# NikolausDemmel/rootba

Measured on NVIDIA H100. Metric: ms/LM-iter (linearize+QR+PCG) on BAL at 1/2/4/8 H100 vs CPU ref, lower is better.
Workload: dtype f32

## Files before the change

rootba_b200/csrc/assembled.cuh:

```cuda
#pragma once

#include "kernels.cuh"

namespace rba {

template <class S>
__global__ void __launch_bounds__(256) k_rcs_terms(const S* __restrict__ panel, const AsmTerm* __restrict__ terms, long long nt,
                                                   int damping, S* __restrict__ stage, const int* __restrict__ done) {
  using V2 = typename ST<S>::V2;
  if (*done) return;
  const int lane = threadIdx.x & 31;
  const int g = lane / 9, p = lane - 9 * g;
  if (lane >= 27) return;
  const long long warps = (long long)gridDim.x * (blockDim.x >> 5);
  for (long long w = 3 * (blockIdx.x * (long long)(blockDim.x >> 5) + (threadIdx.x >> 5)) + g; w < nt; w += 3 * warps) {
    const AsmTerm at = terms[w];
    const int n = at.meta & 0x7fff, lg = (at.meta >> 15) & 7, KP = at.meta >> 18, G = 1 << lg;
    const int ia = at.ij & 0xffff, ib = at.ij >> 16;
    const int ca = 9 * ia + p, pa = ca >> 1;
    const int off_a = 2 * ((pa >> lg) * 32 + (pa & (G - 1))) + (ca & 1);
    const int cb0 = 9 * ib, pb0 = cb0 >> 1;
    const bool odd = cb0 & 1;
    int off_b[5];
#pragma unroll
    for (int k = 0; k < 5; ++k) off_b[k] = ((pb0 + k) >> lg) * 32 + ((pb0 + k) & (G - 1));
    const size_t rstride = (size_t)KP * 64;
    const S* __restrict__ lmp = panel + at.base;
    const int r0 = damping ? 2 * n - 3 : 0, r1 = damping ? 2 * n : 2 * n - 3;
    S acc[9];
#pragma unroll
    for (int q = 0; q < 9; ++q) acc[q] = 0;
#pragma unroll 3
    for (int r = r0; r < r1; ++r) {
      const S* row = lmp + (size_t)r * rstride;
      const V2* row2 = reinterpret_cast<const V2*>(row);
      const S va = __ldg(row + off_a);
      V2 b[5];
#pragma unroll
      for (int k = 0; k < 5; ++k) b[k] = __ldg(row2 + off_b[k]);
      const S el[10] = {b[0].x, b[0].y, b[1].x, b[1].y, b[2].x, b[2].y, b[3].x, b[3].y, b[4].x, b[4].y};
#pragma unroll
      for (int q = 0; q < 9; ++q) acc[q] = fma(va, odd ? el[q + 1] : el[q], acc[q]);
    }
    S* o = stage + 81 * (size_t)w + 9 * p;
#pragma unroll
    for (int q = 0; q < 9; ++q) o[q] = acc[q];
  }
}

template <class S>
__global__ void k_rcs_combine(const int* __restrict__ blk_ptr, const int* __restrict__ wpos, int nblk, const S* __restrict__ stage,
                              S* __restrict__ out, const int* __restrict__ done) {
  if (*done) return;
  const long long i = blockIdx.x * (long long)blockDim.x + threadIdx.x;
  if (i >= 81LL * nblk) return;
  const int bi = (int)(i / 81), e = (int)(i - 81LL * bi);
  const S* st = stage + e;
  S s = 0;
  for (int t = blk_ptr[bi]; t < blk_ptr[bi + 1]; ++t) s += st[81 * (size_t)wpos[t]];
  out[i] = s;
}

constexpr int DMP_WARPS = 4;
constexpr int DMP_BATCH = 16;
template <class S>
__global__ void __launch_bounds__(DMP_WARPS * 32) k_rcs_damping(const int* __restrict__ blk_ptr, const int2* __restrict__ terms, int nblk,
                                                                 const S* __restrict__ dmp, const S* __restrict__ base,
                                                                 const int2* __restrict__ pos, S* __restrict__ out,
                                                                 const int* __restrict__ done) {
  constexpr int B = DMP_BATCH, NV = 28 * sizeof(S) / 16;
  constexpr int ROUNDS = (2 * B * NV + 31) / 32;
  __shared__ __align__(16) S rec[DMP_WARPS][B][2][28];
  if (*done) return;
  const int w = threadIdx.x >> 5, lane = threadIdx.x & 31;
  const int bi = blockIdx.x * DMP_WARPS + w;
  if (bi >= nblk) return;
  const bool own = lane < 27;
  const int p = lane / 3, q = 3 * (lane - 3 * p);
  S s[3] = {0, 0, 0};
  if (own) {
#pragma unroll
    for (int u = 0; u < 3; ++u) s[u] = base[81 * (size_t)bi + 3 * lane + u];
  }
  int4* rv = reinterpret_cast<int4*>(&rec[w][0][0][0]);
  const int t1 = blk_ptr[bi + 1];
  for (int t0 = blk_ptr[bi]; t0 < t1; t0 += B) {
    const int nb = min(B, t1 - t0);
    int4 v[ROUNDS];
#pragma unroll
    for (int c = 0; c < ROUNDS; ++c) {
      const int i = lane + 32 * c, r = i / NV, k = i - r * NV;
      v[c] = make_int4(0, 0, 0, 0);
      if (i < 2 * nb * NV) {
        const int2 tt = __ldg(terms + t0 + (r >> 1));
        v[c] = __ldg(reinterpret_cast<const int4*>(dmp + 28 * (size_t)(r & 1 ? tt.y : tt.x)) + k);
      }
    }
#pragma unroll
    for (int c = 0; c < ROUNDS; ++c)
      if (lane + 32 * c < 2 * nb * NV) rv[lane + 32 * c] = v[c];
    __syncwarp();
    if (own) {
      for (int j = 0; j < nb; ++j) {
        const S* a = rec[w][j][0];
        const S* b = rec[w][j][1];
#pragma unroll
        for (int u = 0; u < 3; ++u) {
          S t = fma(a[p], b[q + u], S(0));
          t = fma(a[9 + p], b[9 + q + u], t);
          t = fma(a[18 + p], b[18 + q + u], t);
          s[u] += t;
        }
      }
    }
    __syncwarp();
  }
  if (own) {
    S* o = out + 81 * (size_t)pos[bi].x + 3 * lane;
#pragma unroll
    for (int u = 0; u < 3; ++u) o[u] = s[u];
  }
}

template <class S>
__global__ void k_rcs_mirror(const int2* __restrict__ pos, int nblk, S* val, const int* __restrict__ done) {
  if (*done) return;
  const long long i = blockIdx.x * (long long)blockDim.x + threadIdx.x;
  if (i >= 81LL * nblk) return;
  const int bi = (int)(i / 81), e = (int)(i - 81LL * bi);
// ... 140 lines not shown
```

rootba_b200/csrc/layout.hpp:

```cpp
#pragma once

#include <algorithm>
#include <cmath>
#include <cstdint>
#include <limits>
#include <numeric>
#include <string>
#include <utility>
#include <vector>

namespace rba {

struct TileInfo {
  long long panel_off;
  int slot_base;
  int lm_base;
  short n;
  short G;
  short KP;
  short nvalid;
};

struct MatvecItem {
  int tile;
// ... 237 lines not shown
    if (!L.csr_y_is_obs) build_csr(nc, L.nyslots, ycam, L.csr_y);
    L.pb_cam_item_ptr.assign(nc + 1, 0);
    for (int c = 0; c < nc; ++c) {
      L.pb_cam_item_ptr[c] = (int)L.pb_items.size();
      for (int b = L.csr_obs.cam_ptr[c]; b < L.csr_obs.cam_ptr[c + 1]; b += PB_SEG_LEN)
        L.pb_items.push_back({c, b, std::min(b + PB_SEG_LEN, L.csr_obs.cam_ptr[c + 1])});
    }
    L.pb_cam_item_ptr[nc] = (int)L.pb_items.size();
  }
  for (const TileInfo& T : L.tiles) {
    const int W = 32 / T.G;
    const int CS = (2 * T.G * T.KP) | 1;
    L.k4_scratch_per_warp = std::max(L.k4_scratch_per_warp, T.KP > kp_max ? 2 * 64 * (int)T.KP : W * CS);
  }
  return "";
}

struct IntPair {
  int x, y;
};

struct PairList {
  std::vector<int> slot0, nn;
  std::vector<IntPair> blk_cam;
  std::vector<int> blk_ptr;
  std::vector<IntPair> terms;
  std::vector<int> wpos;
};

inline std::string build_pair_list(const Layout& L, PairList& P) {
  const int nl = L.nl_local, nc = L.nc;
  P = PairList();
  P.slot0.resize(nl); P.nn.resize(nl);
  long long nt = 0;
  for (int lm = 0; lm < nl; ++lm) {
    const int sidx = L.sorted_of_lm[lm];
    const TileInfo& T = L.tiles[L.tile_of_sorted[sidx]];
    P.slot0[lm] = T.slot_base + (sidx - T.lm_base) * T.n;
    P.nn[lm] = T.n;
    nt += (long long)T.n * (T.n + 1) / 2;
  }
  if (nt > std::numeric_limits<int>::max()) return "more than 2^31 camera-pair terms";
  std::vector<IntPair> raw;
  raw.reserve((size_t)nt);
  for (int lm = 0; lm < nl; ++lm)
    for (int a = 0; a < P.nn[lm]; ++a)
      for (int b = 0; b <= a; ++b) raw.push_back({P.slot0[lm] + a, P.slot0[lm] + b});
  std::vector<int> idx(raw.size()), tmp(raw.size());
  std::iota(idx.begin(), idx.end(), 0);
  std::vector<long long> cnt((size_t)nc + 1);
  auto pass = [&](const std::vector<int>& src, std::vector<int>& dst, bool by_a) {
    std::fill(cnt.begin(), cnt.end(), 0LL);
    for (int w : src) ++cnt[L.slot_cam[by_a ? raw[w].x : raw[w].y] + 1];
    for (int c = 0; c < nc; ++c) cnt[c + 1] += cnt[c];
    for (int w : src) dst[cnt[L.slot_cam[by_a ? raw[w].x : raw[w].y]]++] = w;
  };
  pass(idx, tmp, false);
  pass(tmp, idx, true);
  tmp.clear(); tmp.shrink_to_fit();
  P.terms.resize(raw.size());
  for (size_t t = 0; t < idx.size(); ++t) P.terms[t] = raw[idx[t]];
  P.wpos.swap(idx);
  for (size_t t = 0; t < P.terms.size(); ++t) {
    const IntPair cc{L.slot_cam[P.terms[t].x], L.slot_cam[P.terms[t].y]};
    if (t == 0 || cc.x != P.blk_cam.back().x || cc.y != P.blk_cam.back().y) {
      P.blk_cam.push_back(cc);
      P.blk_ptr.push_back((int)t);
    }
  }
  P.blk_ptr.push_back((int)P.terms.size());
  return "";
}

struct AsmTerm {
  long long base;
  int ij, meta;
};
inline AsmTerm pack_asm_term(long long base, int ia, int ib, int n, int G, int KP) {
  int lg = 0;
  while ((1 << lg) < G) ++lg;
  return {base, ia | ib << 16, n | lg << 15 | KP << 18};
}

constexpr long long ASM_STAGE_BYTES = (long long)2 << 30;

inline int asm_switch_iteration(long long nt, long long panel_scalars, long long s_bytes, int scalar_size) {
  const double staged = 4.0 * (double)nt * 81 * scalar_size, saved = (double)panel_scalars * scalar_size - (double)s_bytes;
  return 1 + (int)std::ceil(2.0 * staged / std::max(saved, 1.0));
}

constexpr int SPMV_CLASSES = 4;
constexpr int SPMV_STAGE_BYTES = 32 * 81 * 4;
constexpr int spmv_chunk_blocks(int scalar_size) { return SPMV_STAGE_BYTES / (81 * scalar_size); }
struct SpmvChunk {
  int row, kb, ke;
  int flags;
};
constexpr int SPMV_FIRST = 1, SPMV_LAST = 2;
struct SpmvDeal {
  int ctas = 0;
  std::vector<int> chunk_ptr;
  std::vector<SpmvChunk> chunks;
};
inline void deal_spmv(const std::vector<int>& row_ptr, int ctas, int chunk_blocks, SpmvDeal& D) {
  D = SpmvDeal();
  const int nrows = (int)row_ptr.size() - 1;
  D.ctas = std::max(1, std::min(ctas, nrows));
  std::vector<long long> cost((size_t)std::max(nrows, 0));
  for (int r = 0; r < nrows; ++r) cost[r] = row_ptr[r + 1] - row_ptr[r];
  const std::vector<int> order = deal_lpt(cost, D.ctas);
  D.chunk_ptr.assign((size_t)D.ctas + 1, 0);
  for (int b = 0; b < D.ctas; ++b) {
    D.chunk_ptr[b] = (int)D.chunks.size();
    for (size_t k = b; k < order.size(); k += D.ctas) {
      const int r = order[k];
      if (r < 0) break;
      const int k0 = row_ptr[r], k1 = row_ptr[r + 1];
      int kb = k0;
      do {
        const int ke = std::min(k1, kb + chunk_blocks);
        D.chunks.push_back({r, kb, ke, (kb == k0 ? SPMV_FIRST : 0) | (ke == k1 ? SPMV_LAST : 0)});
        kb = ke;
      } while (kb < k1);
    }
  }
  D.chunk_ptr[D.ctas] = (int)D.chunks.size();
}

struct AsmPlan {
  long long nt = 0, nblk = 0, nnzb = 0, s_bytes = 0, device_bytes = 0;
  bool fits = false;
  int switch_iteration = 0;
  std::vector<int> row_ptr;
  std::vector<int> col;
  std::vector<IntPair> pos;
  std::vector<AsmTerm> terms;
  SpmvDeal spmv;
};

inline void plan_assembled(const Layout& L, const PairList& P, int scalar_size, AsmPlan& A, int spmv_ctas = 0) {
  A = AsmPlan();
  const int nc = L.nc;
  A.nblk = (long long)P.blk_cam.size();
  A.nt = (long long)P.terms.size();
  long long ndiag = 0;
  for (const IntPair& c : P.blk_cam) ndiag += c.x == c.y;
  A.nnzb = 2 * A.nblk - ndiag;
  A.s_bytes = A.nnzb * 81 * scalar_size;
  A.switch_iteration = asm_switch_iteration(A.nt, L.panel_scalars, A.s_bytes, scalar_size);
  A.fits = 4 * A.s_bytes <= L.panel_scalars * scalar_size && 81 * A.nt * scalar_size <= ASM_STAGE_BYTES;
  if (!A.fits) return;
  A.device_bytes = A.s_bytes + 16 + (A.nblk + A.nt) * 81 * scalar_size + A.nt * (long long)(sizeof(AsmTerm) + sizeof(int) + sizeof(IntPair)) +
                   (A.nblk + 1 + A.nnzb) * (long long)sizeof(int) + A.nblk * (long long)sizeof(IntPair);
  A.row_ptr.assign((size_t)nc + 1, 0);
  A.col.resize((size_t)A.nnzb);
  for (const IntPair& c : P.blk_cam) { ++A.row_ptr[c.x + 1]; if (c.x != c.y) ++A.row_ptr[c.y + 1]; }
  for (int c = 0; c < nc; ++c) A.row_ptr[c + 1] += A.row_ptr[c];
  std::vector<int> fill(A.row_ptr.begin(), A.row_ptr.end() - 1);
  A.pos.resize((size_t)A.nblk);
  for (long long b = 0; b < A.nblk; ++b) {
    const IntPair c = P.blk_cam[b];
    const int lo = fill[c.x]++;
    A.col[lo] = c.y;
    int up = -1;
    if (c.x != c.y) { up = fill[c.y]++; A.col[up] = c.x; }
    A.pos[b] = {lo, up};
  }
  A.terms.reserve((size_t)A.nt);
  for (int lm = 0; lm < L.nl_local; ++lm) {
    const int sidx = L.sorted_of_lm[lm];
    const TileInfo& T = L.tiles[L.tile_of_sorted[sidx]];
    const int g = sidx - T.lm_base;
    for (int a = 0; a < T.n; ++a)
      for (int b = 0; b <= a; ++b) A.terms.push_back(pack_asm_term(T.panel_off + 2LL * g * T.G, a, b, T.n, T.G, T.KP));
  }
  if (spmv_ctas > 0) {
    deal_spmv(A.row_ptr, spmv_ctas, spmv_chunk_blocks(scalar_size), A.spmv);
    A.device_bytes += (long long)A.spmv.chunks.size() * (long long)sizeof(SpmvChunk) + (A.spmv.ctas + 1) * (long long)sizeof(int);
  }
}

}
```

rootba_b200/csrc/solver.cu:

```cuda
#include <cuda_runtime.h>
#include <dlfcn.h>

#include <cstdio>
#include <cstdlib>
#include <cstring>
#include <chrono>
#include <array>
#include <limits>
#include <memory>
#include <string>
#include <utility>
#include <vector>

#include "../../include/rootba_b200.h"
#include "../host/bal_io_fast.hpp"
#include "kernels.cuh"
#include "covariance.cuh"
#include "assembled.cuh"
#include "rigs.cuh"
#include "nccl_dyn.hpp"

namespace rba {

thread_local std::string g_err;
// ... 47 lines not shown
  virtual int set_intrinsics_groups(const int32_t* group) = 0;
  virtual int set_camera_rigs(const int32_t* rig, const void* cam_from_rig) = 0;
  virtual int set_observation_info(const void* sqrt_info) = 0;
  virtual int set_observation_loss(const uint8_t* kind, const void* scale) = 0;
  virtual int set_prior_loss(int32_t prior_kind, int32_t num, const uint8_t* kind, const void* scale) = 0;
  virtual int get_prior_residuals(int32_t prior_kind, void* residual, void* robust_weight) = 0;
  virtual int get_observation_residuals(void* residual, void* robust_weight, uint8_t* flags) = 0;
  virtual int compute_error(rba_residual_info* out) = 0;
  virtual int linearize() = 0;
  virtual int solve(double lambda, void* inc_out, rba_cg_summary* cg) = 0;
  virtual int apply(const void* inc, void* l_diff_out, bool update_cameras) = 0;
  virtual int lm_step(bool linearize_first, double lambda, rba_lm_step_result* out) = 0;
  virtual int lm_run(const rba_lm_opts* o, int max_steps, rba_lm_iteration* log, int* steps_done, int* terminated, rba_stage_timings* totals) = 0;
  virtual int get_timings(rba_stage_timings* out) const = 0;
  virtual int get_stats(rba_workload_stats* out) const = 0;
  virtual int get_scaling(void* scaling, void* diag2) = 0;
  virtual int get_rhs(void* b) = 0;
  virtual int get_precond(void* inv, void* blocks) = 0;
  virtual int right_multiply(const void* x, void* y) = 0;
  virtual int debug_get_block(int lm, void* out, int rows, int cols, void* jls) = 0;
  virtual int compute_covariance(double* cam_cov, double* lm_cov) = 0;
  virtual int compute_covariance_blocks(const rba_covariance_query* q) = 0;
  virtual int time_matvec(int reps, double* sec) = 0;
  virtual int timer_start() = 0;
  virtual int timer_stop(double* sec) = 0;
  virtual void* stream_ptr() = 0;
  virtual int synchronize() = 0;
  virtual int comm_init(const void* uid) = 0;
  virtual int ipc_export(void* out128) = 0;
  virtual int ipc_import(const void* all) = 0;
};

namespace rba {

template <class S>
struct Solver : rba_handle {
  static constexpr int EBLOCKS = 592;
  static constexpr int KPMAX = sizeof(S) == 4 ? 16 : 10;
  static constexpr int TILE_WARPS = 4;
  static constexpr int K1_CAP = 3904;
  static constexpr int K2_CAP = 3072;
  static constexpr int K4_WARPS = 4;
  static constexpr int K4_NS = 2;
  static constexpr int K4_STAGE = 4608;
  static constexpr size_t K4_SMEM_TMA = (size_t)K4_WARPS * K4_NS * K4_STAGE;
  static constexpr long long K4_ITEM_COST = 48;
  static constexpr int IMP_WARPS = 2, IMP_MAXSLOTS = 64, IMP_NS = 1;

  rba_solver_opts opt{};
  KOpts ko{};
  Layout L;
  int nc = 0, nl_total = 0;
  long long nobs_total = 0;
  int device = 0;
  int sm_count = 132;
  cudaStream_t stream = nullptr;
  std::vector<DeviceBuffer<char>> owned;
  size_t device_bytes = 0;
  DevPtrs<S> D{};
  S* cams_bk = nullptr; S* lms_bk = nullptr;
  long long state_version = 0;
  rba_residual_info error_cache{}; long long error_cache_version = -1, error_enqueue_version = -1; bool error_cache_valid = false;
  bool error_enqueued = false;
  int* d_csr_obs_slots = nullptr; ReduceItem* d_csr_obs_items = nullptr; int* d_csr_obs_item_ptr = nullptr;
  int* d_csr_y_slots = nullptr; ReduceItem* d_csr_y_items = nullptr; int* d_csr_y_item_ptr = nullptr;
  int n_obs_items = 0, n_y_items = 0;
  const int* op_slots = nullptr; const ReduceItem* op_items = nullptr; const int* op_item_ptr = nullptr; int n_op_items = 0;
  bool panels = true;
  ReduceItem* d_pb_items = nullptr; int* d_pb_item_ptr = nullptr; int n_pb_items = 0;
  Scratch<S> k1_sc{}, k2_sc{};
  size_t k1_smem = 0, k2_smem = 0;
  int k1_max_blocks = 264, k2_max_blocks = 264;
  TileOrder order_k1{nullptr, 0}, order_kp{nullptr, 0};
  MatvecItem* d_items = nullptr;
  int n_dealt = 0, tma_grid = 1;
  size_t k4_smem_small = 0;
  int imp_tile_split = 0;
  size_t imp_smem = 0; int imp_grid = 1;
  int pcg_cluster = 16;
  bool pcg_partials = true;
  bool peer_ar = true;
  bool asm_hook = true;
  int asm_at = 0;
  int* h_prog = nullptr; int* d_prog = nullptr;
  int pcg_solve_id = 0;
  double* d_epart = nullptr;
  double* d_red = nullptr;
  int* d_flags = nullptr;
  int* d_cam_cnt = nullptr;
  PcgState* d_state = nullptr;
  PcgState* h_state = nullptr;
  struct PinnedResults {
    double error[6];
    int error_flags[4];
    int linearize_flags[4];
    double l_diff;
    int apply_flags[4];
  };
  PinnedResults* h_res = nullptr;
  cudaEvent_t poll_ev[2] = {nullptr, nullptr};
  bool linearized = false;
  bool new_linearization_point = false;
  bool have_inc = false;
  S last_lambda = 0;
  bool damping_valid = false;
  struct HeldTerm {
    std::vector<uint8_t> host;
    DeviceBuffer<uint8_t> flags;
    bool all = false;
  } held;
  struct PriorLoss {
    bool on = false;
    DeviceBuffer<S> rec;
    DeviceBuffer<S> Lw;
  };
  struct CameraPriorTerm {
    bool on = false;
    PriorLoss loss;
    DeviceBuffer<S> mean;
    DeviceBuffer<S> L;
    DeviceBuffer<S> A;
    DeviceBuffer<S> r;
    DeviceBuffer<S> H;
    DeviceBuffer<S> g;
    void adopt(CameraPriorTerm& o) { mean.take(o.mean); L.take(o.L); A.take(o.A); r.take(o.r); H.take(o.H); g.take(o.g); }
  } cprior;
  struct PairPriorTerm {
    int n = 0;
    std::vector<int> item_of;
    PriorLoss loss;
    DeviceBuffer<int> ij;
    DeviceBuffer<S> mean;
    DeviceBuffer<S> L;
    DeviceBuffer<S> A;
    DeviceBuffer<S> r;
    DeviceBuffer<int> item;
    DeviceBuffer<int> nbr;
    DeviceBuffer<S> O;
    DeviceBuffer<int> ptr;
    DeviceBuffer<S> ov;
    void adopt(PairPriorTerm& o) { ij.take(o.ij); mean.take(o.mean); L.take(o.L); A.take(o.A); r.take(o.r); item.take(o.item);
                                   nbr.take(o.nbr); O.take(o.O); ptr.take(o.ptr); ov.take(o.ov); }
  } pprior;
  struct LandmarkPriorTerm {
    int n = 0;
    std::vector<int> item_of;
    PriorLoss loss;
    DeviceBuffer<int> slot;
    DeviceBuffer<int> of_lm;
    DeviceBuffer<int> lm;
    DeviceBuffer<S> mean, L, Lg;
    void adopt(LandmarkPriorTerm& o) { slot.take(o.slot); of_lm.take(o.of_lm); lm.take(o.lm); mean.take(o.mean); L.take(o.L); Lg.take(o.Lg); }
  } lprior;
  struct GroupTerm {
    int n = 0;
    std::vector<int> host_lead;
    DeviceBuffer<int> lead, ptr, mem;
    DeviceBuffer<uint8_t> fixed;
    DeviceBuffer<S> ve, y;
    void adopt(GroupTerm& o) { lead.take(o.lead); ptr.take(o.ptr); mem.take(o.mem); fixed.take(o.fixed); ve.take(o.ve); y.take(o.y); }
  } grp;
  struct RigTerm {
    int n = 0;
    std::vector<int> host_lead;
    DeviceBuffer<int> lead, ptr, mem;
    DeviceBuffer<S> adj;
    DeviceBuffer<double> M;
    DeviceBuffer<S> pt;
    DeviceBuffer<S> du;
    DeviceBuffer<uint8_t> fixed;
    DeviceBuffer<S> ve, y;
    void adopt(RigTerm& o) { lead.take(o.lead); ptr.take(o.ptr); mem.take(o.mem); adj.take(o.adj); M.take(o.M); pt.take(o.pt);
                             du.take(o.du); fixed.take(o.fixed); ve.take(o.ve); y.take(o.y); }
  } rig;
  struct ObservationTerm {
    bool on = false;
    DeviceBuffer<S> W;
    bool loss_on = false;
    DeviceBuffer<S> loss;
  } obs;
  rba_stage_timings tm{};
  EventPair ev_stage1, ev_stage2, ev_precond, ev_pcg, ev_backsub, ev_update, ev_error, ev_mv, ev_user;
  long long launches = 0;
  long long lin_l0 = 0, solve_l0 = 0, apply_l0 = 0;
  NcclApi* nccl = nullptr;
  ncclComm_t comm = nullptr;
  char* peer_mem = nullptr;
  size_t peer_bytes = 0;
  PeerComm pc{};
  bool peer_ok = false;
  int ar_seq = 0, c_seq = 0, s_seq = 0;
  std::vector<void*> ipc_opened;
  bool cov_ready = false;
  int cov_nblk = 0;
  IntPair* d_cov_blk_cam = nullptr; int* d_cov_blk_ptr = nullptr; IntPair* d_cov_terms = nullptr;
  int* d_cov_lm_slot0 = nullptr; int* d_cov_lm_n = nullptr;
  bool asm_on = false, su_valid = false, s_valid = false, su_new = false;
  int asm_nblk = 0, asm_switch = 0; long long asm_nt = 0, asm_nnzb = 0;
  AsmTerm* d_asm_terms = nullptr; int* d_asm_wpos = nullptr; int* d_asm_blk_ptr = nullptr; IntPair* d_asm_pos = nullptr;
  IntPair* d_asm_slots = nullptr;
  int* d_asm_col = nullptr;
  S* d_asm_stage = nullptr; S* d_asm_Su = nullptr; S* d_asm_S = nullptr;
  SpmvChunk* d_spmv_chunks = nullptr; int* d_spmv_chunk_ptr = nullptr; int spmv_grid = 0, spmv_cap = 0;
  bool s_fresh = false;

  ~Solver() override {
    if (comm && nccl) nccl->CommDestroy(comm);
    for (void* p : ipc_opened) cudaIpcCloseMemHandle(p);
    if (h_prog) cudaFreeHost(h_prog);
    if (h_state) cudaFreeHost(h_state);
    if (h_res) cudaFreeHost(h_res);
    for (EventPair* e : {&ev_stage1, &ev_stage2, &ev_precond, &ev_pcg, &ev_backsub, &ev_update, &ev_error, &ev_mv, &ev_user}) {
      if (e->a) cudaEventDestroy(e->a);
      if (e->b) cudaEventDestroy(e->b);
    }
    for (auto& e : poll_ev) if (e) cudaEventDestroy(e);
    if (stream) cudaStreamDestroy(stream);
  }

  template <class T>
  int alloc(DeviceBuffer<T>& b, size_t count, bool zero, bool counted = true) {
    const size_t bytes = std::max<size_t>(count, 1) * sizeof(T);
    void* q = nullptr;
    CU(cudaMalloc(&q, bytes));
    b = DeviceBuffer<T>((T*)q, count);
    if (counted) device_bytes += bytes;
    if (zero) CU(cudaMemsetAsync(q, 0, bytes, stream));
    return RBA_OK;
  }
  template <class T>
  int copy_in(T* dst, const std::vector<T>& v) {
    if (!v.empty()) CU(cudaMemcpyAsync(dst, v.data(), v.size() * sizeof(T), cudaMemcpyHostToDevice, stream));
    return RBA_OK;
  }
  template <class T>
  int dalloc(T** p, size_t count, bool zero = true, bool counted = true) {
    DeviceBuffer<char> b;
    TRY(alloc(b, std::max<size_t>(count, 1) * sizeof(T), zero, counted));
    *p = (T*)b.get();
    owned.push_back(std::move(b));
    return RBA_OK;
  }
  template <class T>
  int upload(T** p, const std::vector<T>& v, bool counted = true) {
    TRY(dalloc(p, v.size(), false, counted));
    return copy_in(*p, v);
  }
  template <class T>
  int fit(DeviceBuffer<T>& next, const DeviceBuffer<T>& cur, size_t count, const std::vector<T>* src = nullptr) {
    if (!cur.get() || cur.size() < count) TRY(alloc(next, count, false));
    return src ? copy_in(next.get() ? next.get() : cur.get(), *src) : RBA_OK;
  }

  int start(EventPair& e) { e.used = true; CU(cudaEventRecord(e.a, stream)); return RBA_OK; }
  int stop(EventPair& e) { CU(cudaEventRecord(e.b, stream)); return RBA_OK; }
  static double elapsed(EventPair& e) {
    if (!e.used) return 0.0;
    float ms = 0;
    if (cudaEventElapsedTime(&ms, e.a, e.b) != cudaSuccess) return 0.0;
    return 1e-3 * ms;
  }

  int init(const rba_problem_view* pv, const rba_solver_opts* o) {
    TRY(validate_options(*o));
    int ndev = 0;
    if (cudaGetDeviceCount(&ndev) != cudaSuccess || ndev == 0) {
      g_err = "no CUDA device: rootba_b200 has no CPU fallback";
      return RBA_ERR_NO_DEVICE;
    }
    if (opt.device >= 0) CU(cudaSetDevice(opt.device));
    CU(cudaGetDevice(&device));
    cudaDeviceProp prop;
    CU(cudaGetDeviceProperties(&prop, device));
    sm_count = prop.multiProcessorCount;
    CU(cudaStreamCreateWithFlags(&stream, cudaStreamNonBlocking));
    for (EventPair* e : {&ev_stage1, &ev_stage2, &ev_precond, &ev_pcg, &ev_backsub, &ev_update, &ev_error, &ev_mv, &ev_user}) {
      CU(cudaEventCreate(&e->a));
      CU(cudaEventCreate(&e->b));
    }
    for (auto& e : poll_ev) CU(cudaEventCreateWithFlags(&e, cudaEventDisableTiming));
    read_test_hooks();
    TRY(upload_layout(pv));
    TRY(deal_work());
    TRY(alloc_buffers());
    TRY(setup_assembled());
    TRY(setup_kernels());
    CU(cudaStreamSynchronize(stream));
    return RBA_OK;
  }

  int validate_options(const rba_solver_opts& o) {
    opt = o;
    if (opt.nranks < 1 || opt.rank < 0 || opt.rank >= opt.nranks) { g_err = "bad rank/nranks"; return RBA_ERR_INVALID_ARGUMENT; }
    if (opt.operator_form != 0 && opt.operator_form != 1) { g_err = "operator_form must be 0 (dense) or 1 (implicit)"; return RBA_ERR_INVALID_ARGUMENT; }
    if (opt.solver_type < 0 || opt.solver_type > 2) { g_err = "solver_type must be 0 (SQUARE_ROOT), 1 (SCHUR_COMPLEMENT) or 2 (POWER_SCHUR_COMPLEMENT)"; return RBA_ERR_INVALID_ARGUMENT; }
    if (opt.solver_type == 2 && opt.nranks > 1) { g_err = "POWER_SCHUR_COMPLEMENT runs on one GPU (the power-series vector kernel has no peer exchange yet)"; return RBA_ERR_UNSUPPORTED; }
    if (opt.stage2_form != 0 && opt.stage2_form != 1) { g_err = "stage2_form must be 0 (Q2 panel, reference) or 1 (orthogonality identity)"; return RBA_ERR_INVALID_ARGUMENT; }
    if (opt.pcg_check_period <= 0) opt.pcg_check_period = 4;
    if (opt.residual_reset_period <= 0) opt.residual_reset_period = 10;
    if (opt.power_order <= 0) opt.power_order = 20;
    panels = opt.operator_form == 0 && opt.solver_type == 0;
    ko.use_valid_projections_only = opt.use_valid_projections_only;
    ko.robust_norm = opt.robust_norm;
    ko.write_panel = panels;
    ko.huber = opt.huber_parameter;
    ko.jacobi_eps = opt.jacobi_scaling_epsilon > 0 ? opt.jacobi_scaling_epsilon : (double)ST<S>::eps_sqrt();
    return RBA_OK;
  }
  bool panel_form() const { return panels && opt.stage2_form == 0; }

  void read_test_hooks() {
    if (const char* e = getenv("RBA_PCG_PARTIALS")) pcg_partials = atoi(e) != 0;
    if (const char* e = getenv("RBA_PCG_CLUSTER")) pcg_cluster = std::max(1, std::min(atoi(e), 16));
    if (const char* e = getenv("RBA_PEER_AR")) peer_ar = atoi(e) != 0;
    if (const char* e = getenv("RBA_ASSEMBLED_RCS")) asm_hook = atoi(e) != 0;
    if (const char* e = getenv("RBA_ASSEMBLED_AT")) asm_at = std::max(0, atoi(e));
    if (const char* e = getenv("RBA_SPMV_CTAS")) spmv_cap = std::max(1, atoi(e));
  }

  int upload_layout(const rba_problem_view* pv) {
    nc = pv->num_cameras;
    nl_total = pv->num_landmarks;
    nobs_total = pv->lm_obs_offset[nl_total];
    std::string msg = build_layout(nc, nl_total, pv->lm_obs_offset, pv->obs_cam_idx, opt.rank, opt.nranks, KPMAX, L);
    if (!msg.empty()) { g_err = msg; return RBA_ERR_INVALID_ARGUMENT; }
    std::vector<S> xy((size_t)2 * L.nslots, S(0));
    const S* src = (const S*)pv->obs_xy;
    for (int s = 0; s < L.nslots; ++s)
      if (L.slot_obs[s] >= 0) { xy[2 * (size_t)s] = src[2 * L.slot_obs[s]]; xy[2 * (size_t)s + 1] = src[2 * L.slot_obs[s] + 1]; }
    TileInfo* d_tiles; int* d_sorted; int* d_slot_cam; int* d_slot_lm; S* d_xy;
    TRY(upload(&d_tiles, L.tiles));
    TRY(upload(&d_sorted, L.sorted_lm));
    TRY(upload(&d_slot_cam, L.slot_cam));
    TRY(upload(&d_slot_lm, L.slot_lm));
    TRY(upload(&d_xy, xy));
    D.tiles = d_tiles; D.ntiles = (int)L.tiles.size(); D.sorted_lm = d_sorted;
    D.slot_cam = d_slot_cam; D.slot_lm = d_slot_lm; D.slot_xy = d_xy; D.nslots = L.nslots; D.nc = nc;
    TRY(upload(&d_csr_obs_slots, L.csr_obs.slots));
    TRY(upload(&d_csr_obs_items, L.csr_obs.items));
    TRY(upload(&d_csr_obs_item_ptr, L.csr_obs.cam_item_ptr));
    n_obs_items = (int)L.csr_obs.items.size();
    if (L.csr_y_is_obs) {
      d_csr_y_slots = d_csr_obs_slots; d_csr_y_items = d_csr_obs_items; d_csr_y_item_ptr = d_csr_obs_item_ptr;
      n_y_items = n_obs_items;
    } else {
      TRY(upload(&d_csr_y_slots, L.csr_y.slots));
      TRY(upload(&d_csr_y_items, L.csr_y.items));
      TRY(upload(&d_csr_y_item_ptr, L.csr_y.cam_item_ptr));
      n_y_items = (int)L.csr_y.items.size();
    }
    if (panels) { op_slots = d_csr_y_slots; op_items = d_csr_y_items; op_item_ptr = d_csr_y_item_ptr; n_op_items = n_y_items; }
    else { op_slots = d_csr_obs_slots; op_items = d_csr_obs_items; op_item_ptr = d_csr_obs_item_ptr; n_op_items = n_obs_items; }
    TRY(upload(&d_pb_items, L.pb_items));
    TRY(upload(&d_pb_item_ptr, L.pb_cam_item_ptr));
    n_pb_items = (int)L.pb_items.size();
    return RBA_OK;
  }

  int deal_work() {
    if (panels) {
      TRY(deal_matvec_items());
    } else {
      while (imp_tile_split < (int)L.tiles.size() && (32 / L.tiles[imp_tile_split].G) * L.tiles[imp_tile_split].n <= IMP_MAXSLOTS) ++imp_tile_split;
      imp_smem = (size_t)IMP_WARPS * IMP_NS * (size_t)IMP_MAXSLOTS * 48 * sizeof(S);
      CU(cudaFuncSetAttribute((k_matvec_implicit_tma<S, IMP_WARPS, IMP_MAXSLOTS, IMP_NS>), cudaFuncAttributeMaxDynamicSharedMemorySize, (int)imp_smem));
      int bps = 0;
      CU(cudaOccupancyMaxActiveBlocksPerMultiprocessor(&bps, (k_matvec_implicit_tma<S, IMP_WARPS, IMP_MAXSLOTS, IMP_NS>), IMP_WARPS * 32, imp_smem));
      imp_grid = std::max(1, std::min((imp_tile_split + IMP_WARPS - 1) / IMP_WARPS, sm_count * std::max(1, bps)));
    }
    long long need1 = 0, need2 = 0;
    for (const TileInfo& T : L.tiles) {
      const int Wn = (32 / T.G) * T.n;
      need1 = std::max<long long>(need1, (long long)Wn * 60 + 64);
      need2 = std::max<long long>(need2, (long long)stage2_need(T.n, T.G, T.KP));
    }
    tile_scratch_geometry(k1_sc, K1_CAP, need1, k1_smem, k1_max_blocks);
    tile_scratch_geometry(k2_sc, K2_CAP, need2, k2_smem, k2_max_blocks);
    TRY(deal_tiles(tile_grid(k1_max_blocks) * TILE_WARPS, order_k1));
    TRY(deal_tiles(tile_grid(sm_count * 8) * TILE_WARPS, order_kp));
    return RBA_OK;
  }

  int deal_matvec_items() {
    CU(cudaFuncSetAttribute((k_matvec_small_tma<S, K4_WARPS, K4_NS, K4_STAGE>), cudaFuncAttributeMaxDynamicSharedMemorySize, (int)K4_SMEM_TMA));
    int occ = 0;
    CU(cudaOccupancyMaxActiveBlocksPerMultiprocessor(&occ, (k_matvec_small_tma<S, K4_WARPS, K4_NS, K4_STAGE>), K4_WARPS * 32, K4_SMEM_TMA));
    int bps = std::max(1, (int)((220 * 1024) / (K4_SMEM_TMA + 1024)));
    if (occ > 0) bps = std::min(bps, occ);
    const int nsmall = (int)L.items.size() - L.n_items_large;
    tma_grid = grid_for(nsmall, K4_WARPS, bps);
    const int W = tma_grid * K4_WARPS;
    std::vector<MatvecItem> items = L.items;
    if (nsmall > W) {
      std::vector<long long> cost(nsmall);
      for (int q = 0; q < nsmall; ++q) {
        const MatvecItem& it = L.items[L.n_items_large + q];
        cost[q] = (long long)it.nrows * L.tiles[it.tile].KP + K4_ITEM_COST;
      }
      const MatvecItem empty{};
      items.resize(L.n_items_large);
// ... 1432 lines not shown

  int get_timings(rba_stage_timings* out) const override { *out = tm; out->kernel_launches = launches; return RBA_OK; }
  int get_stats(rba_workload_stats* out) const override {
    std::memset(out, 0, sizeof(*out));
    out->num_landmarks_local = L.nl_local;
    out->num_observations_local = L.nobs_local;
    out->sum_n2 = L.sum_n2;
    out->max_n = L.max_n;
    out->num_tiles = (int)L.tiles.size();
    out->panel_scalars = L.panel_scalars;
    out->panel_scalars_algorithmic = 18 * L.sum_n2;
    out->device_bytes = (int64_t)device_bytes;
    out->matvec_algorithmic_bytes = handover() == Handover::Assembled ? (81 * asm_nnzb + 18 * (int64_t)nc) * (int64_t)sizeof(S) + 4 * (asm_nnzb + nc + 1)
                                                                        : (18 * L.sum_n2 + 18 * L.nobs_local) * (int64_t)sizeof(S) + 4 * L.nobs_local;
    out->landmark_begin = L.lm_begin;
    out->landmark_end = L.lm_end;
    out->num_matvec_items = (int)L.items.size();
    return RBA_OK;
  }

  int get_scaling(void* scaling, void* diag2) override {
    if (scaling) CU(cudaMemcpyAsync(scaling, D.scaling, (size_t)9 * nc * sizeof(S), cudaMemcpyDeviceToHost, stream));
    if (diag2) CU(cudaMemcpyAsync(diag2, D.diag2, (size_t)9 * nc * sizeof(S), cudaMemcpyDeviceToHost, stream));
    CU(cudaStreamSynchronize(stream));
    return RBA_OK;
  }
  int get_rhs(void* b) override {
    CU(cudaMemcpyAsync(b, D.b, (size_t)9 * nc * sizeof(S), cudaMemcpyDeviceToHost, stream));
    CU(cudaStreamSynchronize(stream));
    return RBA_OK;
  }
  int get_precond(void* inv, void* blocks) override {
    if (inv) CU(cudaMemcpyAsync(inv, D.inv, (size_t)81 * nc * sizeof(S), cudaMemcpyDeviceToHost, stream));
    if (blocks) CU(cudaMemcpyAsync(blocks, D.blocks, (size_t)81 * nc * sizeof(S), cudaMemcpyDeviceToHost, stream));
    CU(cudaStreamSynchronize(stream));
    return RBA_OK;
  }
  int right_multiply(const void* x, void* y) override {
    if (!linearized || !damping_valid) { g_err = "rba_right_multiply needs rba_linearize + rba_solve first"; return RBA_ERR_STATE; }
    CU(cudaMemcpyAsync(D.z, x, (size_t)9 * nc * sizeof(S), cudaMemcpyHostToDevice, stream));
    TRY(matvec_launch(D.z, true));
    TRY(allreduce(D.y, (size_t)9 * nc));
    k_pcg_q<S><<<NPART, 128, 0, stream>>>(D, D.y, D.z, D.y, last_lambda);
    ++launches;
    CU(cudaMemcpyAsync(y, D.y, (size_t)9 * nc * sizeof(S), cudaMemcpyDeviceToHost, stream));
    CU(cudaStreamSynchronize(stream));
    CU(cudaGetLastError());
    return RBA_OK;
  }

  int time_matvec(int reps, double* sec) override {
    if (!linearized || !damping_valid) { g_err = "rba_time_matvec needs rba_linearize + rba_solve first"; return RBA_ERR_STATE; }
    TRY(matvec_launch(D.p, false));
    TRY(start(ev_mv));
    for (int r = 0; r < reps; ++r) TRY(matvec_launch(D.p, false));
    TRY(stop(ev_mv));
    CU(cudaStreamSynchronize(stream));
    CU(cudaGetLastError());
    *sec = elapsed(ev_mv) / std::max(reps, 1);
    tm.matvec_time = *sec;
    return RBA_OK;
  }

  int timer_start() override { return start(ev_user); }
  int timer_stop(double* sec) override {
    int rc = stop(ev_user); if (rc) return rc;
    CU(cudaStreamSynchronize(stream));
    *sec = elapsed(ev_user);
    return RBA_OK;
  }
  void* stream_ptr() override { return (void*)stream; }
  int synchronize() override { CU(cudaStreamSynchronize(stream)); return RBA_OK; }

  bool asm_candidate() const { return asm_hook && opt.nranks == 1 && panels; }
  int setup_assembled() {
    if (!asm_candidate()) return RBA_OK;
    PairList P;
    const std::string msg = build_pair_list(L, P);
    if (!msg.empty()) { g_err = msg; return RBA_ERR_UNSUPPORTED; }
    int occ = 0;
    CU(cudaOccupancyMaxActiveBlocksPerMultiprocessor(&occ, k_rcs_spmv<S>, SPMV_CLASSES * 32, 0));
    AsmPlan A;
    const int ctas = std::max(1, occ) * sm_count;
    plan_assembled(L, P, sizeof(S), A, spmv_cap > 0 ? std::min(spmv_cap, ctas) : ctas);
    if (!A.fits) return RBA_OK;
    size_t free_b = 0, total_b = 0;
    CU(cudaMemGetInfo(&free_b, &total_b));
    if ((size_t)A.device_bytes + ((size_t)256 << 20) > free_b) return RBA_OK;
    TRY(upload(&d_asm_terms, A.terms));
    TRY(upload(&d_asm_wpos, P.wpos));
    TRY(upload(&d_asm_slots, P.terms));
    TRY(upload(&d_asm_blk_ptr, P.blk_ptr));
    TRY(upload(&d_asm_pos, A.pos));
    TRY(upload(&d_asm_col, A.col));
    TRY(upload(&d_spmv_chunks, A.spmv.chunks));
    TRY(upload(&d_spmv_chunk_ptr, A.spmv.chunk_ptr));
    spmv_grid = A.spmv.ctas;
    TRY(dalloc(&d_asm_stage, (size_t)A.nt * 81, false));
    TRY(dalloc(&d_asm_Su, (size_t)A.nblk * 81));
    TRY(dalloc(&d_asm_S, (size_t)A.nnzb * 81 + 16 / sizeof(S)));
    asm_nt = A.nt; asm_nblk = (int)A.nblk; asm_nnzb = A.nnzb;
    asm_switch = asm_at > 0 ? asm_at : A.switch_iteration;
    asm_on = true;
    return RBA_OK;
  }
  void assemble(int damping) {
    const int* done = &d_state->done;
    const unsigned per_entry = (unsigned)((81LL * asm_nblk + 255) / 256);
    if (damping) {
      k_rcs_damping<S><<<(asm_nblk + DMP_WARPS - 1) / DMP_WARPS, DMP_WARPS * 32, 0, stream>>>(
          d_asm_blk_ptr, (const int2*)d_asm_slots, asm_nblk, D.dmp, d_asm_Su, (const int2*)d_asm_pos, d_asm_S, done);
      k_rcs_mirror<S><<<per_entry, 256, 0, stream>>>((const int2*)d_asm_pos, asm_nblk, d_asm_S, done);
    } else {
      const int grid = (int)std::max<long long>(1, std::min<long long>((asm_nt + 23) / 24, (long long)sm_count * 16));
      k_rcs_terms<S><<<grid, 256, 0, stream>>>(D.panel, d_asm_terms, asm_nt, 0, d_asm_stage, done);
      k_rcs_combine<S><<<per_entry, 256, 0, stream>>>(d_asm_blk_ptr, d_asm_wpos, asm_nblk, d_asm_stage, d_asm_Su, done);
    }
    launches += 2;
  }

  int cov_build_lists() {
    if (cov_ready) return RBA_OK;
    PairList P;
    const std::string msg = build_pair_list(L, P);
    if (!msg.empty()) { g_err = msg; return RBA_ERR_UNSUPPORTED; }
    TRY(upload(&d_cov_blk_cam, P.blk_cam, false));
    TRY(upload(&d_cov_blk_ptr, P.blk_ptr, false));
    TRY(upload(&d_cov_terms, P.terms, false));
    TRY(upload(&d_cov_lm_slot0, P.slot0, false));
    TRY(upload(&d_cov_lm_n, P.nn, false));
    cov_nblk = (int)P.blk_cam.size();
    cov_ready = true;
    return RBA_OK;
  }
  template <bool TA, bool TB>
  void cov_gemm(long long M, long long N, long long K, double alpha, const double* A, long long lda, const double* B, long long ldb,
                double beta, double* C, long long ldc, int lower, int ktri) {
    k_cov_dgemm<TA, TB><<<dim3((unsigned)(M / COV_TB), (unsigned)(N / COV_TB)), 256, 0, stream>>>((int)M, (int)N, (int)K, alpha, A, lda, B,
                                                                                                   ldb, beta, C, ldc, lower, ktri);
  }
  int cov_copy(double* dst, long long dld, const double* src, long long sld, long long rows, long long cols) {
    CU(cudaMemcpy2DAsync(dst, dld * sizeof(double), src, sld * sizeof(double), rows * sizeof(double), cols, cudaMemcpyDeviceToDevice, stream));
    return RBA_OK;
  }
  int cov_group_passes(double* A, long long ld, long long n, int expand) {
    k_cov_group_symmetrize<<<dim3((unsigned)((n + 31) / 32), (unsigned)((n + 7) / 8)), dim3(32, 8), 0, stream>>>(A, ld, n);
    for (int columns = 0; columns < 2; ++columns)
      k_cov_group_pass<<<(unsigned)((n + 255) / 256), 256, 0, stream>>>(A, ld, n, groups(), columns, expand);
    CU(cudaGetLastError());
    return RBA_OK;
  }
  int cov_rig_passes(double* A, long long ld, long long n, int expand) {
    k_cov_group_symmetrize<<<dim3((unsigned)((n + 31) / 32), (unsigned)((n + 7) / 8)), dim3(32, 8), 0, stream>>>(A, ld, n);
    for (int columns = 0; columns < 2; ++columns)
      k_cov_rig_pass<S><<<(unsigned)((n + 255) / 256), 256, 0, stream>>>(A, ld, n, rigs(), columns, expand);
    CU(cudaGetLastError());
    return RBA_OK;
  }
  struct CovInverse {
    DeviceBuffer<char> scratch;
    double* A = nullptr;
    double* d = nullptr;
    double* kb = nullptr; double* wl = nullptr; int* rk = nullptr;
    long long np = 0;
  };
  int cov_factor_inverse(const char* fn, const std::vector<size_t>& extra, CovInverse& c, std::vector<char*>& out) {
    if (opt.nranks > 1) {
      g_err = std::string(fn) + ": sharded handles (nranks > 1) are not supported: the reduced camera matrix would need a cross-rank sum";
      return RBA_ERR_UNSUPPORTED;
    }
    TRY(cov_build_lists());
    constexpr long long TB = COV_TB;
    const long long n = 9LL * nc, np = (n + TB - 1) / TB * TB, ns = L.nslots;
    const int nl = L.nl_local, nt = (int)(np / TB), n_lmp = lprior.n;
    size_t total = 0;
    auto carve = [&](size_t bytes) { const size_t o = total; total += (bytes + 255) & ~size_t(255); return o; };
    const size_t o_A = carve((size_t)(np * np) * 8), o_W = carve((size_t)(np * TB) * 8), o_Y = carve((size_t)(np * TB) * 8),
                 o_T = carve((size_t)(TB * TB) * 8), o_d = carve((size_t)np * 8), o_jp = carve((size_t)ns * 18 * 8),
                 o_kb = carve((size_t)ns * 27 * 8), o_wl = carve((size_t)nl * 9 * 8), o_rk = carve((size_t)nl * 4), o_fail = carve(4);
    std::vector<size_t> o_extra;
    for (size_t b : extra) o_extra.push_back(carve(b));
    size_t free_b = 0, total_b = 0;
    CU(cudaMemGetInfo(&free_b, &total_b));
    if (total > free_b) {
      g_err = std::string(fn) + " needs " + std::to_string(total) + " bytes of device memory (a dense " + std::to_string(n) + " x " +
              std::to_string(n) + " float64 reduced camera matrix plus scratch); " + std::to_string(free_b) + " bytes are free";
      return RBA_ERR_UNSUPPORTED;
    }
    TRY(alloc(c.scratch, total, false, false));
    char* base = c.scratch.get();
    double* A = (double*)(base + o_A); double* W = (double*)(base + o_W); double* Y = (double*)(base + o_Y);
    double* Tt = (double*)(base + o_T); double* d = (double*)(base + o_d); double* jp = (double*)(base + o_jp);
    double* kb = (double*)(base + o_kb); double* wl = (double*)(base + o_wl); int* rk = (int*)(base + o_rk);
    int* fail = (int*)(base + o_fail);
    out.clear();
    for (size_t o : o_extra) out.push_back(base + o);
    const int wgrid = std::max(1, std::min((nl + 3) / 4, sm_count * 16));
    c.A = A; c.d = d; c.kb = kb; c.wl = wl; c.rk = rk; c.np = np;
// ... 465 lines not shown
```

Measured before the change: 5.572.

## Stage landmark panel tiles into shared memory via bulk async copy for RCS assembly

Adds a persistent per-SM kernel that computes the reduced camera system outer-product terms tile by tile. Each tile's panel rows are streamed into double-buffered shared memory with mbarrier-tracked bulk copies. Tiles are dealt to CTAs with LPT load balancing, and each thread computes three 9-wide rows of a term instead of one. The goal is to replace repeated global/L2 panel reads with shared-memory reuse and to overlap loads with compute. The trade-off is one CTA per SM with large shared memory, sqrt-based index decoding, and a per-term stage scatter through a shared buffer.

Result: faster. 5.461 (median of 6 runs) (-2.0%).

```diff
diff --git a/rootba_b200/csrc/assembled.cuh b/rootba_b200/csrc/assembled.cuh
--- a/rootba_b200/csrc/assembled.cuh
+++ b/rootba_b200/csrc/assembled.cuh
@@ -45,6 +45,118 @@
     S* o = stage + 81 * (size_t)w + 9 * p;
 #pragma unroll
     for (int q = 0; q < 9; ++q) o[q] = acc[q];
+  }
+}
+
+template <class S>
+__device__ __forceinline__ void rcs_tile_terms(const S* P, const AsmTile& T, const int* __restrict__ lm_term0, S* out,
+                                               S* __restrict__ stage) {
+  using V2 = typename ST<S>::V2;
+  constexpr int NW = RCS_OUT_BYTES / (32 * 27 * (int)sizeof(S));
+  const int w = threadIdx.x >> 5, lane = threadIdx.x & 31;
+  const int n = T.n, lg = T.lg, G = 1 << lg, nv = T.nvalid, R = 2 * n - 3, rs = T.KP * 64;
+  const int items = 3 * (n * (n + 1) / 2) * nv;
+  for (int i0 = 32 * w; i0 < items; i0 += 32 * NW) {
+    const int it = i0 + lane;
+    int dst = -1;
+    if (it < items) {
+      const int g = it % nv, rest = it / nv, k = rest / 3, u = rest - 3 * k;
+      int a = (int)((sqrtf(8.f * k + 1.f) - 1.f) * 0.5f);
+      while (a * (a + 1) / 2 > k) --a;
+      while ((a + 1) * (a + 2) / 2 <= k) ++a;
+      const int b = k - a * (a + 1) / 2;
+      const int lb = g * G;
+      int off_a[3];
+#pragma unroll
+      for (int e = 0; e < 3; ++e) {
+        const int c = 9 * a + 3 * u + e, pc = c >> 1;
+        off_a[e] = 2 * ((pc >> lg) * 32 + lb + (pc & (G - 1))) + (c & 1);
+      }
+      const int cb0 = 9 * b, pb0 = cb0 >> 1;
+      const bool odd = cb0 & 1;
+      int off_b[5];
+#pragma unroll
+      for (int kk = 0; kk < 5; ++kk) off_b[kk] = ((pb0 + kk) >> lg) * 32 + lb + ((pb0 + kk) & (G - 1));
+      S acc[3][9];
+#pragma unroll
+      for (int e = 0; e < 3; ++e)
+#pragma unroll
+        for (int q = 0; q < 9; ++q) acc[e][q] = 0;
+#pragma unroll 2
+      for (int r = 0; r < R; ++r) {
+        const S* row = P + (size_t)r * rs;
+        const V2* row2 = reinterpret_cast<const V2*>(row);
+        S va[3];
+#pragma unroll
+        for (int e = 0; e < 3; ++e) va[e] = row[off_a[e]];
+        V2 bv[5];
+#pragma unroll
+        for (int kk = 0; kk < 5; ++kk) bv[kk] = row2[off_b[kk]];
+        const S el[10] = {bv[0].x, bv[0].y, bv[1].x, bv[1].y, bv[2].x, bv[2].y, bv[3].x, bv[3].y, bv[4].x, bv[4].y};
+#pragma unroll
+        for (int e = 0; e < 3; ++e)
+#pragma unroll
+          for (int q = 0; q < 9; ++q) acc[e][q] = fma(va[e], odd ? el[q + 1] : el[q], acc[e][q]);
+      }
+#pragma unroll
+      for (int e = 0; e < 3; ++e)
+#pragma unroll
+        for (int q = 0; q < 9; ++q) out[27 * lane + 9 * e + q] = acc[e][q];
+      dst = 81 * (lm_term0[T.lm_base + g] + k) + 27 * u;
+    }
+    __syncwarp();
+#pragma unroll 9
+    for (int j = lane; j < 32 * 27; j += 32) {
+      const int src = j / 27;
+      const int d = __shfl_sync(0xffffffffu, dst, src);
+      if (d >= 0) stage[(size_t)d + j - 27 * src] = out[j];
+    }
+    __syncwarp();
+  }
+}
+
+template <class S>
+__global__ void __launch_bounds__(RCS_OUT_BYTES / (27 * sizeof(S)), 1) k_rcs_tiles(const S* __restrict__ panel, const AsmTile* __restrict__ tiles,
+                                                                  const int* __restrict__ tile_ptr, const int* __restrict__ lm_term0,
+                                                                  S* __restrict__ stage, const int* __restrict__ done) {
+  constexpr int SB = (RCS_SMEM_BYTES - RCS_OUT_BYTES) / RCS_NS / 256 * 256;
+  extern __shared__ __align__(128) unsigned char rcs_smem[];
+  constexpr int NW = RCS_OUT_BYTES / (32 * 27 * (int)sizeof(S));
+  __shared__ __align__(8) uint64_t bars[RCS_NS];
+  __shared__ int out_of[RCS_NS];
+  if (*done) return;
+  const int c0 = tile_ptr[blockIdx.x], nt = tile_ptr[blockIdx.x + 1] - c0;
+  if (threadIdx.x == 0) {
+    for (int s = 0; s < RCS_NS; ++s) {
+      mbar_init(&bars[s], 1);
+      out_of[s] = 0;
+    }
+    mbar_fence_init();
+  }
+  __syncthreads();
+  const uint64_t policy = l2_evict_first_policy();
+  auto span = [&](const AsmTile& T) { return (2 * T.n - 3) * T.KP * 64 * (int)sizeof(S); };
+  auto request = [&](int i) {
+    const AsmTile T = tiles[c0 + i];
+    const int s = i % RCS_NS, bytes = span(T) <= SB ? span(T) : 0;
+    mbar_expect_tx(&bars[s], (uint32_t)bytes);
+    if (bytes) bulk_g2s(rcs_smem + (size_t)s * SB, panel + T.panel_off, (uint32_t)bytes, &bars[s], policy);
+  };
+  if (threadIdx.x == 0)
+    for (int i = 0; i < min(nt, RCS_NS); ++i) request(i);
+  S* out = reinterpret_cast<S*>(rcs_smem + (size_t)RCS_NS * SB) + (threadIdx.x >> 5) * 32 * 27;
+  for (int i = 0; i < nt; ++i) {
+    const AsmTile T = tiles[c0 + i];
+    mbar_wait(&bars[i % RCS_NS], (i / RCS_NS) & 1u);
+    if (span(T) <= SB)
+      rcs_tile_terms<S>(reinterpret_cast<const S*>(rcs_smem + (size_t)(i % RCS_NS) * SB), T, lm_term0, out, stage);
+    else
+      rcs_tile_terms<S>(panel + T.panel_off, T, lm_term0, out, stage);
+    if ((threadIdx.x & 31) == 0 && atomicAdd(&out_of[i % RCS_NS], 1) == NW - 1) {
+      out_of[i % RCS_NS] = 0;
+      if (i + RCS_NS < nt) request(i + RCS_NS);
+    }
+    __syncwarp();
   }
 }
 
diff --git a/rootba_b200/csrc/layout.hpp b/rootba_b200/csrc/layout.hpp
--- a/rootba_b200/csrc/layout.hpp
+++ b/rootba_b200/csrc/layout.hpp
@@ -343,6 +343,17 @@
   return {base, ia | ib << 16, n | lg << 15 | KP << 18};
 }
 
+constexpr int RCS_NS = 2;
+constexpr int RCS_SMEM_BYTES = 227 * 1024 - 1024;
+constexpr int RCS_OUT_BYTES = 16 * 32 * 27 * 4;
+constexpr int rcs_warps(int scalar_size) { return RCS_OUT_BYTES / (32 * 27 * scalar_size); }
+constexpr int rcs_stage_bytes() { return (RCS_SMEM_BYTES - RCS_OUT_BYTES) / RCS_NS / 256 * 256; }
+struct AsmTile {
+  long long panel_off;
+  int lm_base;
+  short n, lg, KP, nvalid;
+};
+
 constexpr long long ASM_STAGE_BYTES = (long long)2 << 30;
 
 inline int asm_switch_iteration(long long nt, long long panel_scalars, long long s_bytes, int scalar_size) {
@@ -397,9 +408,12 @@
   std::vector<IntPair> pos;
   std::vector<AsmTerm> terms;
   SpmvDeal spmv;
-};
-
-inline void plan_assembled(const Layout& L, const PairList& P, int scalar_size, AsmPlan& A, int spmv_ctas = 0) {
+  std::vector<int> tile_ptr;
+  std::vector<AsmTile> tiles;
+  std::vector<int> lm_term0;
+};
+
+inline void plan_assembled(const Layout& L, const PairList& P, int scalar_size, AsmPlan& A, int spmv_ctas = 0, int tile_ctas = 0) {
   A = AsmPlan();
   const int nc = L.nc;
   A.nblk = (long long)P.blk_cam.size();
@@ -439,6 +453,31 @@
     deal_spmv(A.row_ptr, spmv_ctas, spmv_chunk_blocks(scalar_size), A.spmv);
     A.device_bytes += (long long)A.spmv.chunks.size() * (long long)sizeof(SpmvChunk) + (A.spmv.ctas + 1) * (long long)sizeof(int);
   }
-}
-
-}
+  if (tile_ctas > 0) {
+    A.lm_term0.assign(L.sorted_lm.size(), -1);
+    for (int lm = 0, t0 = 0; lm < L.nl_local; ++lm) {
+      const int sidx = L.sorted_of_lm[lm], n = L.tiles[L.tile_of_sorted[sidx]].n;
+      A.lm_term0[sidx] = t0;
+      t0 += n * (n + 1) / 2;
+    }
+    std::vector<AsmTile> all;
+    std::vector<long long> cost;
+    for (const TileInfo& T : L.tiles) {
+      short lg = 0;
+      while ((1 << lg) < T.G) ++lg;
+      all.push_back({T.panel_off, T.lm_base, T.n, lg, T.KP, T.nvalid});
+      cost.push_back((long long)2 * T.n * T.n * (T.n + 1) / 2 * T.nvalid);
+    }
+    const int ctas = std::max(1, std::min<int>(tile_ctas, (int)all.size()));
+    const std::vector<int> order = deal_lpt(cost, ctas);
+    A.tile_ptr.assign((size_t)ctas + 1, 0);
+    for (int b = 0; b < ctas; ++b) {
+      A.tile_ptr[b] = (int)A.tiles.size();
+      for (size_t k = b; k < order.size() && order[k] >= 0; k += ctas) A.tiles.push_back(all[order[k]]);
+    }
+    A.tile_ptr[ctas] = (int)A.tiles.size();
+    A.device_bytes += (long long)A.tiles.size() * (long long)sizeof(AsmTile) + (long long)(A.tile_ptr.size() + A.lm_term0.size()) * (long long)sizeof(int);
+  }
+}
+
+}
diff --git a/rootba_b200/csrc/solver.cu b/rootba_b200/csrc/solver.cu
--- a/rootba_b200/csrc/solver.cu
+++ b/rootba_b200/csrc/solver.cu
@@ -153,6 +153,7 @@
   bool peer_ar = true;
   bool asm_hook = true;
   int asm_at = 0;
+  bool rcs_tiles_hook = true;
   int* h_prog = nullptr; int* d_prog = nullptr;
   int pcg_solve_id = 0;
   double* d_epart = nullptr;
@@ -272,6 +273,7 @@
   IntPair* d_asm_slots = nullptr;
   int* d_asm_col = nullptr;
   S* d_asm_stage = nullptr; S* d_asm_Su = nullptr; S* d_asm_S = nullptr;
+  AsmTile* d_rcs_tiles = nullptr; int* d_rcs_tile_ptr = nullptr; int* d_rcs_lm_term0 = nullptr; int rcs_grid = 0;
   SpmvChunk* d_spmv_chunks = nullptr; int* d_spmv_chunk_ptr = nullptr; int spmv_grid = 0, spmv_cap = 0;
   bool s_fresh = false;
 
@@ -387,6 +389,7 @@
     if (const char* e = getenv("RBA_ASSEMBLED_RCS")) asm_hook = atoi(e) != 0;
     if (const char* e = getenv("RBA_ASSEMBLED_AT")) asm_at = std::max(0, atoi(e));
     if (const char* e = getenv("RBA_SPMV_CTAS")) spmv_cap = std::max(1, atoi(e));
+    if (const char* e = getenv("RBA_RCS_TILES")) rcs_tiles_hook = atoi(e) != 0;
   }
 
   int upload_layout(const rba_problem_view* pv) {
@@ -1985,12 +1988,13 @@
     CU(cudaOccupancyMaxActiveBlocksPerMultiprocessor(&occ, k_rcs_spmv<S>, SPMV_CLASSES * 32, 0));
     AsmPlan A;
     const int ctas = std::max(1, occ) * sm_count;
-    plan_assembled(L, P, sizeof(S), A, spmv_cap > 0 ? std::min(spmv_cap, ctas) : ctas);
+    CU(cudaFuncSetAttribute(k_rcs_tiles<S>, cudaFuncAttributeMaxDynamicSharedMemorySize, RCS_NS * rcs_stage_bytes() + RCS_OUT_BYTES));
+    plan_assembled(L, P, sizeof(S), A, spmv_cap > 0 ? std::min(spmv_cap, ctas) : ctas, rcs_tiles_hook ? sm_count : 0);
     if (!A.fits) return RBA_OK;
     size_t free_b = 0, total_b = 0;
     CU(cudaMemGetInfo(&free_b, &total_b));
     if ((size_t)A.device_bytes + ((size_t)256 << 20) > free_b) return RBA_OK;
-    TRY(upload(&d_asm_terms, A.terms));
+    if (!rcs_tiles_hook) TRY(upload(&d_asm_terms, A.terms));
     TRY(upload(&d_asm_wpos, P.wpos));
     TRY(upload(&d_asm_slots, P.terms));
     TRY(upload(&d_asm_blk_ptr, P.blk_ptr));
@@ -1999,6 +2003,12 @@
     TRY(upload(&d_spmv_chunks, A.spmv.chunks));
     TRY(upload(&d_spmv_chunk_ptr, A.spmv.chunk_ptr));
     spmv_grid = A.spmv.ctas;
+    if (rcs_tiles_hook) {
+      TRY(upload(&d_rcs_tiles, A.tiles));
+      TRY(upload(&d_rcs_tile_ptr, A.tile_ptr));
+      TRY(upload(&d_rcs_lm_term0, A.lm_term0));
+      rcs_grid = (int)A.tile_ptr.size() - 1;
+    }
     TRY(dalloc(&d_asm_stage, (size_t)A.nt * 81, false));
     TRY(dalloc(&d_asm_Su, (size_t)A.nblk * 81));
     TRY(dalloc(&d_asm_S, (size_t)A.nnzb * 81 + 16 / sizeof(S)));
@@ -2015,8 +2025,12 @@
           d_asm_blk_ptr, (const int2*)d_asm_slots, asm_nblk, D.dmp, d_asm_Su, (const int2*)d_asm_pos, d_asm_S, done);
       k_rcs_mirror<S><<<per_entry, 256, 0, stream>>>((const int2*)d_asm_pos, asm_nblk, d_asm_S, done);
     } else {
-      const int grid = (int)std::max<long long>(1, std::min<long long>((asm_nt + 23) / 24, (long long)sm_count * 16));
-      k_rcs_terms<S><<<grid, 256, 0, stream>>>(D.panel, d_asm_terms, asm_nt, 0, d_asm_stage, done);
+      if (rcs_grid > 0) {
+        k_rcs_tiles<S><<<rcs_grid, rcs_warps(sizeof(S)) * 32, RCS_NS * rcs_stage_bytes() + RCS_OUT_BYTES, stream>>>(D.panel, d_rcs_tiles, d_rcs_tile_ptr, d_rcs_lm_term0, d_asm_stage, done);
+      } else {
+        const int grid = (int)std::max<long long>(1, std::min<long long>((asm_nt + 23) / 24, (long long)sm_count * 16));
+        k_rcs_terms<S><<<grid, 256, 0, stream>>>(D.panel, d_asm_terms, asm_nt, 0, d_asm_stage, done);
+      }
       k_rcs_combine<S><<<per_entry, 256, 0, stream>>>(d_asm_blk_ptr, d_asm_wpos, asm_nblk, d_asm_stage, d_asm_Su, done);
     }
     launches += 2;
```
